# PointCloudLibrary/pcl

Hardware: AMD Instinct MI355X
Metric: ICP correspondences/sec (higher is better)
Workload: dtype f32 search / f64 accumulate

## Files before the change

### __graft_entry__.py

```python
import os
import subprocess
import sys

ROOT = os.path.dirname(os.path.abspath(__file__))
if ROOT not in sys.path:
    sys.path.insert(0, ROOT)


def build():
    env = dict(os.environ)
    env.setdefault("HIPCC", "/opt/rocm/bin/hipcc")
    subprocess.check_call(["make", "-C", os.path.join(ROOT, "pcl_amd", "csrc"), "-j8"], env=env)
    if subprocess.call(["bash", os.path.join(ROOT, "scripts", "build_variant.sh"), "verify", "-DPCLHIP_VERIFY_BOUNDS"], env=env,
                       stdout=subprocess.DEVNULL) != 0:
        print("warning: the verify-bounds variant did not build (tests/test_gpu_verify_bounds.py will skip)", file=sys.stderr)
    subprocess.check_call(["make", "-C", os.path.join(ROOT, "oracle")])
    if os.path.exists("/opt/rocm/lib/llvm/bin/clang++"):
        subprocess.check_call(["make", "-C", os.path.join(ROOT, "tests", "wavesim"), "-j8"], stdout=subprocess.DEVNULL)
    import pcl_amd
    from pcl_amd import _lib
    _lib.load()


def smoke():
    import numpy as np

    import pcl_amd
    from oracle import pcl_oracle as orc

    n = 20000
    tgt, src, T_gt = pcl_amd.synth.icp_pair(n)
    ctx = pcl_amd.Context(0)
    tree = pcl_amd.KdTree(ctx)
    tree.setInputCloud(tgt)
    gi, gd = tree.nearestKSearch(src[:4096], 8)
    otree = orc.KdTree(tgt)
    oi, od = otree.knn(src[:4096], 8)
    assert np.array_equal(gi, oi) and np.array_equal(gd, od), "k-NN mismatch vs oracle"
    ne = pcl_amd.NormalEstimation(ctx)
    ne.setInputCloud(tgt)
    ne.setSearchMethod(tree)
    ne.setKSearch(8)
    ne.setViewPoint(0, 0, 10)
    nrm = ne.compute()
    onrm, _ = otree.normals(tgt, 8, viewpoint=(0, 0, 10))
    assert np.abs(np.sum(nrm[:, :3] * onrm[:, :3], axis=1)).min() > 1 - 1e-4, "normals mismatch"
    icp = pcl_amd.IterativeClosestPointWithNormals(ctx)
    icp.setSearchMethodTarget(tree)
# ... 20 lines not shown
```

### pcl_amd/csrc/search.hip

```cpp
#include <hip/hip_runtime.h>

#include <type_traits>

#include <cfloat>
#include <cmath>
#include <cstdlib>
#include <cstring>

#include "traverse.hpp"
#include "standoff.hpp"
#include "normals_math.hpp"
#include "device_scan.hpp"
#include "icp_xform.hpp"
#include <mutex>
#include <unordered_map>
#include <vector>

namespace pclhip {

constexpr int BLOCK = 256;
constexpr int WAVES_PER_BLOCK = BLOCK / WAVE;
constexpr uint32_t COLD_RUN = 4;

#define KNN_MINW(K) ((K) <= 8 ? 4 : 1)
template <int K>
using KnnWaveLds = WaveLdsBoxT<(K == 1 ? 3072 : LEAF_BATCH * LEAF_FLOATS * 4)>;
template <int K>
__global__ __launch_bounds__(BLOCK, KNN_MINW(K)) void knn_reg_kernel(IndexView ix, const float4* __restrict__ q,
                                                        uint32_t nq, int k, int32_t* __restrict__ out_idx,
                                                        float* __restrict__ out_d2, unsigned long long* gstats) {
  __shared__ KnnWaveLds<K> wl_s[WAVES_PER_BLOCK];
  __shared__ Box topbox_s[TOPCACHE_BOXES];
  load_top_cache(ix, topbox_s);
  const int lane = threadIdx.x & (WAVE - 1);
  const uint32_t ngroups = (nq + WAVE - 1) / WAVE;
  const GroupSchedule sched(ngroups);
  TraverseStats ts;
  GroupFeed feed(sched, ix.sched_ctr);
  for (uint32_t gl = feed.first(sched); gl != GroupFeed::END; gl = feed.advance()) {
    const uint32_t g = sched.global(gl);
    if (g >= ngroups) break;
    feed.ahead(gl);
    const uint32_t i = g * WAVE + lane;
    float4 p = make_float4(0, 0, 0, 0);
    bool valid = i < nq;
    if (valid) p = q[i];
    const uint32_t oq = __float_as_uint(p.w);
    const bool real = valid;
    valid = valid && isfinite(p.x) && isfinite(p.y) && isfinite(p.z);
    const float qx[1] = {p.x}, qy[1] = {p.y}, qz[1] = {p.z};
    const bool vv[1] = {valid};
    if constexpr (K == 1) {
      NN1Min fast;
      fast.init(__builtin_inff());
      traverse<NN1Min, true>(ix, qx, qy, qz, vv, fast, wl_s[threadIdx.x / WAVE], topbox_s, ts);
// ... 716 lines not shown
__device__ __forceinline__ void icp_search_body(const IndexView& ix, float4* __restrict__ cur,
                                                const float4* __restrict__ src0, uint32_t ns, Mat34 T,
                                                const IcpControl* __restrict__ ctl, const RegionBox& region, int order,
                                                float bound, int flags, uint32_t* __restrict__ match_pos,
                                                uint32_t* __restrict__ match, float* __restrict__ match_d2,
                                                unsigned long long* gstats, IcpWaveLds* wl_s, Box* topbox_s,
                                                const OG& og = OG()) {
  static_assert(!OWNED || Q == 1, "served-group lists are per 64-point group");
  bool restart = false;
  if (ctl != nullptr) {
    if (ctl->stop != 0) return;
    restart = ctl->restart != 0;
    if ((flags & 4) != 0 && !restart) return;
#pragma unroll
    for (int i = 0; i < 12; ++i) T.m[i] = ctl->T_apply[i];
  }
  const float4* in = restart ? src0 : cur;
  const int use_max = flags & 1;
  load_top_cache(ix, topbox_s);
  const int lane = threadIdx.x & (WAVE - 1);
  const int wave = threadIdx.x / WAVE;
  const uint32_t GROUP = (Q == 1 && !OWNED) ? search_fill_of(flags) : uint32_t(WAVE * Q);
  const bool lane_in_group = (Q != 1 || OWNED) ? true : uint32_t(threadIdx.x & (WAVE - 1)) < GROUP;
  uint32_t ngroups = (ns + GROUP - 1) / GROUP;
  uint32_t epoch = 0;
  if constexpr (OWNED) {
    ngroups = og.count[0];
    epoch = og.state->epoch;
  }
  const auto gid = [&](uint32_t slot) -> uint32_t {
    if constexpr (OWNED) return slot < ngroups ? og.list[slot] : 0u;
    else return slot;
  };
  const GroupSchedule sched(ngroups);
  TraverseStats ts;
  uint32_t gl = sched.first();
  uint32_t g = (gl < sched.end()) ? sched.global(gl) : ngroups;
  GroupFeed feed(sched, ix.sched_ctr);
  const auto next_now = [&](uint32_t from) -> uint32_t {
    uint32_t out = GroupFeed::END;
    if (from == GroupFeed::END) return out;
    if (!feed.static_next(from, out)) {
      feed.request();
      out = feed.resolve();
    }
    return out;
  };
  constexpr bool deep = DEEP;
  uint32_t gl_next = (gl < sched.end()) ? next_now(gl) : GroupFeed::END;
  uint32_t gl_nn = deep ? next_now(gl_next) : GroupFeed::END;
  float4 p_n[Q], t_n[Q];
  uint32_t sp_n[Q], sp_nn[Q];
  uint32_t gid_n = gid(g), st_n = 0;
  if constexpr (OWNED) st_n = (g < ngroups && !restart) ? (og.stamp[gid_n] & 0x7FFFFFFFu) : 0u;
  {
    const uint32_t g1 = (gl_next != GroupFeed::END) ? sched.global(gl_next) : ngroups;
    const uint32_t gid1 = gid(g1);
#pragma unroll
    for (int q = 0; q < Q; ++q) {
      p_n[q] = make_float4(0, 0, 0, 0);
      t_n[q] = make_float4(0, 0, 0, 0);
      sp_n[q] = NO_INDEX;
      sp_nn[q] = NO_INDEX;
      const uint32_t i = gid_n * GROUP + q * WAVE + lane;
      if (g < ngroups && i < ns && lane_in_group) {
        p_n[q] = (OWNED && st_n == 0u) ? src0[i] : in[i];
        sp_n[q] = restart ? NO_INDEX : match_pos[i];
      }
      const uint32_t i1 = gid1 * GROUP + q * WAVE + lane;
      if (g1 < ngroups && i1 < ns && lane_in_group) sp_nn[q] = restart ? NO_INDEX : match_pos[i1];
      if (sp_n[q] != NO_INDEX) t_n[q] = ix.pts[sp_n[q]];
    }
  }
#ifdef PCLHIP_ICP_PROFILE
  uint64_t icp_t = clock64();
#define ICP_LAP(i)                              \
  do {                                          \
    const uint64_t icp_now = clock64();         \
    ts.c[i] += uint32_t(icp_now - icp_t);       \
    icp_t = icp_now;                            \
  } while (0)
#else
#define ICP_LAP(i) (void)0
#endif
  while (g < ngroups) {
    float4 p[Q], t0[Q];
    uint32_t seed_pos[Q];
    bool in_range[Q], valid[Q];
    float qx[Q], qy[Q], qz[Q];
    const uint32_t gcur = gid_n, st_cur = st_n;
#pragma unroll
    for (int q = 0; q < Q; ++q) {
      p[q] = p_n[q];
      t0[q] = t_n[q];
      seed_pos[q] = sp_n[q];
      in_range[q] = lane_in_group && (gcur * GROUP + q * WAVE + lane) < ns;
    }
    const uint32_t g2 = (gl_next != GroupFeed::END) ? sched.global(gl_next) : ngroups;
    const uint32_t g3 = (gl_nn != GroupFeed::END) ? sched.global(gl_nn) : ngroups;
    gid_n = gid(g2);
    const uint32_t gid_nn = gid(g3);
    if constexpr (OWNED) st_n = (g2 < ngroups && !restart) ? (og.stamp[gid_n] & 0x7FFFFFFFu) : 0u;
    uint32_t gl_after = GroupFeed::END;
    bool asked = false;
    const uint32_t gl_last = deep ? gl_nn : gl_next;
    if (gl_last != GroupFeed::END && !feed.static_next(gl_last, gl_after)) {
      feed.request();
      asked = true;
    }
    bool next_ok[Q];
#pragma unroll
    for (int q = 0; q < Q; ++q) {
      const uint32_t i2 = gid_n * GROUP + q * WAVE + lane;
      next_ok[q] = g2 < ngroups && i2 < ns && lane_in_group;
      p_n[q] = make_float4(0, 0, 0, 0);
      t_n[q] = make_float4(0, 0, 0, 0);
      if (deep) {
        sp_n[q] = sp_nn[q];
        if (next_ok[q]) {
          p_n[q] = (OWNED && st_n == 0u) ? src0[i2] : in[i2];
          if (sp_n[q] != NO_INDEX) t_n[q] = ix.pts[sp_n[q]];
        }
        const uint32_t i3 = gid_nn * GROUP + q * WAVE + lane;
        sp_nn[q] = NO_INDEX;
        if (g3 < ngroups && i3 < ns && lane_in_group) sp_nn[q] = restart ? NO_INDEX : match_pos[i3];
      } else {
        sp_n[q] = NO_INDEX;
        if (next_ok[q]) {
          p_n[q] = (OWNED && st_n == 0u) ? src0[i2] : in[i2];
          sp_n[q] = restart ? NO_INDEX : match_pos[i2];
        }
      }
    }
    NN1MinT<Q> fast;
    fast.init(bound);
#pragma unroll
    for (int q = 0; q < Q; ++q) {
      valid[q] = in_range[q] && isfinite(p[q].x) && isfinite(p[q].y) && isfinite(p[q].z);
      if (valid[q]) {
        if constexpr (OWNED) own_replay(og.state, st_cur, restart ? 0u : epoch, order, p[q]);
// ... 49 lines not shown
    }
#pragma unroll
    for (int q = 0; q < Q; ++q) {
      NN1 pol;
      pol.soa = ix.soa;
      pol.key = KEY_NONE;
      pol.pos = fast.bestpos[q];
      if (fast.bestpos[q] != NO_INDEX) {
        const float w = (fast.bestpos[q] == seed_pos[q]) ? t0[q].w : ix.pts[fast.bestpos[q]].w;
        pol.key = make_key(fast.best[q], __float_as_uint(w));
      }
      const bool redo[1] = {valid[q] && (fast.tie[q] || (fast.bestpos[q] == NO_INDEX && !use_max))};
      if (__builtin_amdgcn_ballot_w64(redo[0]) != 0) {
        NN1 ex = pol;
        const float ex_x[1] = {qx[q]}, ex_y[1] = {qy[q]}, ex_z[1] = {qz[q]};
        traverse<NN1, SPARSE>(ix, ex_x, ex_y, ex_z, redo, ex, wl_s[wave], topbox_s, ts);
        if (redo[0]) pol = ex;
      }
      const uint32_t mid = key_index(pol.key);
      const bool found = valid[q] && mid != NO_INDEX;
      if (in_range[q]) {
        const uint32_t i = gcur * GROUP + q * WAVE + lane;
        match[i] = found ? mid : NO_INDEX;
        match_pos[i] = found ? pol.pos : NO_INDEX;
        match_d2[i] = found ? key_dist(pol.key) : __builtin_inff();
      }
    }
    if constexpr (OWNED) {
      if (lane == 0) og.stamp[gcur] = epoch + 1u;
    }
    g = g2;
    if (deep) {
      gl_next = gl_nn;
      gl_nn = asked ? feed.resolve() : gl_after;
    } else {
      gl_next = asked ? feed.resolve() : gl_after;
    }
    ICP_LAP(7);
  }
#undef ICP_LAP
  flush_stats(ts, gstats);
}

template <bool OWNED = false, class OG = NoOwnedGroups>
__device__ __forceinline__ void icp_cold_search_body(const IndexView& ix, float4* __restrict__ cur,
                                                     const float4* __restrict__ src0, uint32_t ns, Mat34 T,
                                                     const IcpControl* __restrict__ ctl, const RegionBox& region, int order,
                                                     float bound, int flags, float so_from,
                                                     uint32_t* __restrict__ match_pos, uint32_t* __restrict__ match,
                                                     float* __restrict__ match_d2, unsigned long long* gstats,
                                                     IcpWaveLds* wl_s, Box* topbox_s, const OG& og = OG()) {
  bool restart = false;
  if (ctl != nullptr) {
    if (ctl->stop != 0) return;
    restart = true;
#pragma unroll
    for (int i = 0; i < 12; ++i) T.m[i] = ctl->T_apply[i];
  }
  const float4* in = restart ? src0 : cur;
  const int use_max = flags & 1;
  load_top_cache(ix, topbox_s);
  const int lane = threadIdx.x & (WAVE - 1);
  const int wave = threadIdx.x / WAVE;
  const uint32_t GF = OWNED ? uint32_t(WAVE) : search_fill_of(flags);
  const bool lane_in_group = uint32_t(lane) < GF;
  uint32_t ngroups = (ns + GF - 1) / GF;
  if constexpr (OWNED) ngroups = og.count[0];
  const auto gid = [&](uint32_t slot) -> uint32_t {
    if constexpr (OWNED) return slot < ngroups ? og.list[slot] : 0u;
    else return slot;
  };
  TraverseStats ts;
  PrevGroup prev;
  prev.init();
  const GroupSchedule sched(ngroups);
  constexpr uint32_t RUN = COLD_RUN;
  const uint32_t nruns = (sched.groups_per_xcd + RUN - 1u) / RUN;
  uint32_t* const run_ctr = ix.sched_ctr + (blockIdx.x % (gridDim.x < 8u ? gridDim.x : 8u)) * uint32_t(SCHED_CTR_STRIDE);
  for (uint32_t run = sched.slot_wave; run < nruns;) {
  uint32_t ticket = 0;
  if (lane == 0) ticket = atomicAdd(run_ctr, 1u);
  prev.forget();
  uint32_t gl = run * RUN;
  const uint32_t run_end = (gl + RUN) < sched.groups_per_xcd ? (gl + RUN) : sched.groups_per_xcd;
  float4 p_n = make_float4(0, 0, 0, 0);
  {
    const uint32_t g0 = (gl < run_end) ? sched.global(gl) : ngroups;
    if (g0 < ngroups && lane_in_group && gid(g0) * GF + lane < ns) p_n = in[gid(g0) * GF + lane];
  }
  for (; gl < run_end; ++gl) {
    const uint32_t g = sched.global(gl);
    if (g >= ngroups) break;
    float4 p = p_n;
    const uint32_t i = gid(g) * GF + lane;
    const bool in_range = lane_in_group && i < ns;
    {
      const uint32_t g2 = (gl + 1u < run_end) ? sched.global(gl + 1u) : ngroups;
      p_n = make_float4(0, 0, 0, 0);
      if (g2 < ngroups && lane_in_group && gid(g2) * GF + lane < ns) p_n = in[gid(g2) * GF + lane];
    }
    if constexpr (OWNED) {
      if (lane == 0) og.stamp[gid(g)] = 1u;
    }
    NN1Min fast;
    fast.init(bound);
    bool valid = in_range && isfinite(p.x) && isfinite(p.y) && isfinite(p.z);
    if (valid) {
      const float x = xform_row(T.m[0], T.m[1], T.m[2], T.m[3], p.x, p.y, p.z, order);
      const float y = xform_row(T.m[4], T.m[5], T.m[6], T.m[7], p.x, p.y, p.z, order);
      const float z = xform_row(T.m[8], T.m[9], T.m[10], T.m[11], p.x, p.y, p.z, order);
      p.x = x; p.y = y; p.z = z;
      cur[i] = p;
      if (region.on) valid = in_region(region, x, y, z);
    } else if (in_range && restart) {
      cur[i] = p;
    }
    const float qx[1] = {p.x}, qy[1] = {p.y}, qz[1] = {p.z};
    const bool vv[1] = {valid};
    uint32_t hint = NO_INDEX;
    const bool done =
        standoff_search(ix, p.x, p.y, p.z, valid, fast, wl_s[wave], topbox_s, ts, prev, (flags & 2) != 0, so_from, hint);
    prev.outcome(done);
#if defined(PCLHIP_SO_PROFILE) || defined(PCLHIP_SO_REASONS)
    const uint64_t so_t0 = clock64();
    TraverseStats ts_fb;
#else
    TraverseStats& ts_fb = ts;
#endif
    if (!done) traverse<NN1Min, true>(ix, qx, qy, qz, vv, fast, wl_s[wave], topbox_s, ts_fb, (flags & 2) ? hint : NO_INDEX, true);
    fast.resolve(ix, qx, qy, qz);
    NN1 pol;
    pol.soa = ix.soa;
    pol.key = KEY_NONE;
    pol.pos = fast.bestpos[0];
    if (fast.bestpos[0] != NO_INDEX) pol.key = make_key(fast.best[0], __float_as_uint(ix.pts[fast.bestpos[0]].w));
    {
      const bool redo[1] = {valid && (fast.tie[0] || (fast.bestpos[0] == NO_INDEX && !use_max))};
      if (__builtin_amdgcn_ballot_w64(redo[0]) != 0) {
        NN1 ex = pol;
        traverse<NN1, true>(ix, qx, qy, qz, redo, ex, wl_s[wave], topbox_s, ts_fb);
        if (redo[0]) pol = ex;
      }
    }
    const uint32_t mid = key_index(pol.key);
    const bool found = valid && mid != NO_INDEX;
    if (in_range) {
      match[i] = found ? mid : NO_INDEX;
      match_pos[i] = found ? pol.pos : NO_INDEX;
      match_d2[i] = found ? key_dist(pol.key) : __builtin_inff();
    }
    prev.record(p.x, p.y, p.z, found ? pol.pos : NO_INDEX);
#if defined(PCLHIP_SO_PROFILE)
    ts.c[7] += uint32_t(clock64() - so_t0);
    if (!done) ++ts.c[4];
#elif defined(PCLHIP_SO_REASONS)
    (void)so_t0;
    if (!done) ++ts.c[4];
#endif
  }
  run = sched.waves_per_xcd + uniform_u32(ticket);
  }
  flush_stats(ts, gstats);
}

template <int MINW, int Q, bool SPARSE, bool DEEP = false>
__global__ __launch_bounds__(BLOCK, MINW) void icp_search_kernel(IndexView ix, float4* __restrict__ cur,
                                                                 const float4* __restrict__ src0, uint32_t ns,
                                                                 Mat34 T, const IcpControl* __restrict__ ctl,
                                                                 RegionBox region, int order, float bound, int flags,
                                                                 uint32_t* __restrict__ match_pos,
                                                                 uint32_t* __restrict__ match,
                                                                 float* __restrict__ match_d2,
                                                                 unsigned long long* gstats
                                                                 ) {
  __shared__ IcpWaveLds wl_s[WAVES_PER_BLOCK];
  __shared__ Box topbox_s[TOPCACHE_BOXES];
  icp_search_body<Q, SPARSE, false, NoOwnedGroups, DEEP>(ix, cur, src0, ns, T, ctl, region, order, bound, flags, match_pos, match,
                                                         match_d2, gstats, wl_s, topbox_s);
}

#ifndef PCLHIP_COLD_MINW
#define PCLHIP_COLD_MINW 4
#endif
__global__ __launch_bounds__(BLOCK, PCLHIP_COLD_MINW) void icp_cold_search_kernel(
    IndexView ix, float4* __restrict__ cur, const float4* __restrict__ src0, uint32_t ns, Mat34 T,
    const IcpControl* __restrict__ ctl, RegionBox region, int order, float bound, int flags, float so_from,
    uint32_t* __restrict__ match_pos, uint32_t* __restrict__ match, float* __restrict__ match_d2, unsigned long long* gstats) {
  __shared__ IcpWaveLds wl_s[WAVES_PER_BLOCK];
  __shared__ Box topbox_s[TOPCACHE_BOXES];
  icp_cold_search_body(ix, cur, src0, ns, T, ctl, region, order, bound, flags, so_from, match_pos, match, match_d2, gstats,
                       wl_s, topbox_s);
}

template <bool DEEP>
// ... 758 lines not shown
    }
    (void)hipEventRecord(device_loop ? ev[0] : icp->ev0, s);
    if (lane_now && !device_loop) {
    } else if (owned) {
      hipLaunchKernelGGL(icp_own_flag_kernel, dim3((ngroups + BLOCK - 1) / BLOCK), dim3(BLOCK), 0, s, ctl, icp->own_state,
                         icp->own_gbox, icp->region, ngroups, icp->n, icp->own_stamp, icp->own_flags, icp->own_prefix, icp->match,
                         icp->match_pos, icp->match_d2);
      hipLaunchKernelGGL(icp_own_list_kernel, dim3((ngroups + OWN_CHUNK - 1) / OWN_CHUNK), dim3(BLOCK), 0, s, ctl, icp->own_state,
                         icp->own_flags, icp->own_prefix, ngroups, icp->own_list, icp->own_tot);
      const int go = resident_blocks(ctx, icp_search_owned_kernel, ngroups);
      PCLHIP_LAUNCH_FED(ctx, icp_search_owned_kernel, dim3(go), dim3(BLOCK), 0, s, v, icp->src_cur, icp->src_sorted0, icp->n, M,
                         ctl, icp->region, order, bound, kflags, so_from, standoff ? 1 : 0, icp->match_pos, icp->match,
                         icp->match_d2, ctx->stats, og);
    } else if (standoff && device_loop) {
      const int gd = resident_blocks(ctx, icp_search_dual_kernel<false>, ngroups);
      if (deep_for(gd, ngroups)) {
        PCLHIP_LAUNCH_FED(ctx, icp_search_dual_kernel<true>, dim3(gd), dim3(BLOCK), 0, s, v, icp->src_cur, icp->src_sorted0, icp->n, M,
                           ctl, icp->region, order, bound, kflags, so_from, icp->match_pos, icp->match, icp->match_d2, ctx->stats);
      } else {
        PCLHIP_LAUNCH_FED(ctx, icp_search_dual_kernel<false>, dim3(gd), dim3(BLOCK), 0, s, v, icp->src_cur, icp->src_sorted0, icp->n, M,
                           ctl, icp->region, order, bound, kflags, so_from, icp->match_pos, icp->match, icp->match_d2, ctx->stats);
      }
    } else if (cold) {
      const int gc = resident_blocks(ctx, icp_cold_search_kernel, ngroups);
      PCLHIP_LAUNCH_FED(ctx, icp_cold_search_kernel, dim3(gc), dim3(BLOCK), 0, s, v, icp->src_cur, icp->src_sorted0, icp->n, M,
                         ctl, icp->region, order, bound, kflags, so_from, icp->match_pos, icp->match, icp->match_d2,
                         ctx->stats);
    } else {
      const int gk = resident_blocks(ctx, ks, ngroups);
      if (deep_for(gk, ngroups)) ks = icp_search_kernel<4, 1, true, true>;
      PCLHIP_LAUNCH_FED(ctx, ks, dim3(gk), dim3(BLOCK), 0, s, v, icp->src_cur, icp->src_sorted0,
                         icp->n, M, ctl, icp->region, order, bound, kflags, icp->match_pos, icp->match, icp->match_d2, ctx->stats);
    }
    if (lane_now) {
      const pclhip_status lst = launch_lane_search(icp, M.m, ctl, order, bound, use_max);
      if (lst != PCLHIP_OK) return lst;
    }
    (void)hipEventRecord(device_loop ? ev[1] : icp->ev_mid, s);
    icp->mid_recorded = true;
    if (icp->search_only && !device_loop) {
      (void)hipEventRecord(icp->ev1, s);
      PCLHIP_CHECK_HIP(ctx, hipGetLastError());
      return PCLHIP_OK;
    }
    const uint8_t* keep = nullptr;
    if (filters) {
      pclhip_status st = apply_correspondence_filters(icp, max_d2, use_max);
      if (st != PCLHIP_OK) return st;
      keep = icp->keep;
    }
    constexpr int acc_per_cu = 4;
    int ga = ctx->num_cus * acc_per_cu;
    if (ga > icp->grid_blocks) ga = icp->grid_blocks;
    {
      const int need = int((uint64_t(icp->n) + 1023u) / 1024u);
      if (ga > need) ga = need < 64 ? 64 : need;
    }
    if (owned && mode == PCLHIP_ICP_POINT_TO_PLANE)
      hipLaunchKernelGGL(icp_accumulate_owned_kernel<PCLHIP_ICP_POINT_TO_PLANE>, dim3(ga), dim3(BLOCK), 0, s, v, icp->src_cur,
                         icp->n, icp->match_pos, icp->match_d2, keep, ctl, icp->enforce_same_direction_normals ? 1 : 0,
                         icp->partials, og);
    else if (owned)
      hipLaunchKernelGGL(icp_accumulate_owned_kernel<PCLHIP_ICP_POINT_TO_POINT>, dim3(ga), dim3(BLOCK), 0, s, v, icp->src_cur,
                         icp->n, icp->match_pos, icp->match_d2, keep, ctl, icp->enforce_same_direction_normals ? 1 : 0,
                         icp->partials, og);
    else if (mode == PCLHIP_ICP_POINT_TO_PLANE)
      launch_accumulate<PCLHIP_ICP_POINT_TO_PLANE>(icp, v, ga, keep, M, ctl, s);
    else if (mode == PCLHIP_ICP_SYMMETRIC)
      launch_accumulate<PCLHIP_ICP_SYMMETRIC>(icp, v, ga, keep, M, ctl, s);
    else
      launch_accumulate<PCLHIP_ICP_POINT_TO_POINT>(icp, v, ga, keep, M, ctl, s);
    (void)hipEventRecord(device_loop ? ev[2] : icp->ev1, s);
    solved = device_loop && !icp_is_sharded(icp);
    hipLaunchKernelGGL(icp_finalize_kernel, dim3(1), dim3(FINALIZE_THREADS), 0, s, icp->partials, ga, icp->sums_dev, ctl,
                       solved ? icp->ctl : static_cast<IcpControl*>(nullptr), icp->steps);
  } else {
    if (device_loop) {
      (void)hipEventRecord(ev[0], s);
      (void)hipEventRecord(ev[1], s);
    }
    if (filters) {
      const pclhip_status es = apply_empty_shard_collectives(icp);
      if (es != PCLHIP_OK) return es;
    }
    PCLHIP_CHECK_HIP(ctx, hipMemsetAsync(icp->sums_dev, 0, NS * sizeof(double), s));
    if (device_loop) (void)hipEventRecord(ev[2], s);
  }
  PCLHIP_CHECK_HIP(ctx, hipGetLastError());
  pclhip_status st = allreduce_record(icp);
// ... 119 lines not shown
  PCLHIP_CHECK_HIP(ctx, e);
  return PCLHIP_OK;
}

int icp_grid_blocks(pclhip_ctx* ctx, uint32_t ns) {
  const uint32_t ngroups = (ns + WAVE - 1) / WAVE;
  int g = resident_blocks(ctx, icp_search_kernel<4, 1, true>, ngroups);
  if (ctx->num_cus * 8 > g) g = ctx->num_cus * 8;
  return g;
}


bool search_built_with_verify_bounds() {
#ifdef PCLHIP_VERIFY_BOUNDS
  return true;
#else
  return false;
#endif
}

void preload_search_kernels(pclhip_ctx* ctx) {
  (void)resident_blocks(ctx, icp_search_kernel<4, 1, true>, 1);
  (void)resident_blocks(ctx, icp_cold_search_kernel, 1);
  (void)resident_blocks(ctx, icp_search_dual_kernel<false>, 1);
  (void)resident_blocks(ctx, icp_search_dual_kernel<true>, 1);
  (void)resident_blocks(ctx, icp_search_kernel<4, 1, true, true>, 1);
  (void)resident_blocks(ctx, normals_kernel<8>, 1);
  (void)resident_blocks(ctx, knn_reg_kernel<1>, 1);
}

}

#include "gicp.hpp"
```

### pcl_amd/csrc/traverse.hpp

```cpp
#pragma once

#include "pclhip_internal.hpp"

namespace pclhip {

constexpr int STACK_ENTRIES = 208;
constexpr int LEAF_BATCH = 16;
#ifndef PCLHIP_PAIR_MODE
#define PCLHIP_PAIR_MODE 1
#endif
constexpr bool pair_mode = PCLHIP_PAIR_MODE != 0;
constexpr int LEAF_FLOATS = 4 * LEAF;

template <int BUF_BYTES>
struct __attribute__((aligned(16))) WaveLdsT {
  static constexpr int BUF_FLOATS = BUF_BYTES / 4;
  static constexpr int LIST_STRIDE = 3;
  uint2 stack[STACK_ENTRIES];
  float4 list[3 * FANOUT];
  float rad[FANOUT];
  float buf[BUF_FLOATS];
  __device__ __forceinline__ float* radii() { return rad; }
};
template <int BUF_BYTES>
// ... 1109 lines not shown
      } else if (alive && lane != jn) {
        const int at = sp + __builtin_popcountll(others & ((1ull << lane) - 1ull));
        stack[at] = make_uint2((cl << 28) | (first + uint32_t(lane)), __float_as_uint(lbG));
      }
      sp += __builtin_popcountll(others);
#ifndef PCLHIP_STATS_LANES
      ts.c[3] += uint32_t(__builtin_popcountll(others));
#endif
      __builtin_amdgcn_wave_barrier();
      level = cl;
      node = first + uint32_t(jn);
      have = true;
    }
  }
}

__device__ __forceinline__ void flush_stats(const TraverseStats& ts_in, unsigned long long* g) {
#ifdef PCLHIP_VERIFY_BOUNDS
  TraverseStats ts = ts_in;
#pragma unroll
  for (int o = 32; o > 0; o >>= 1) {
    ts.c[6] += __shfl_xor(ts.c[6], o);
    ts.c[7] += __shfl_xor(ts.c[7], o);
  }
#else
  const TraverseStats& ts = ts_in;
#endif
  if (g != nullptr && (threadIdx.x & (WAVE - 1)) == 0) {
#pragma unroll
    for (int i = 0; i < 8; ++i) atomicAdd(g + i, (unsigned long long)ts.c[i]);
  }
}

struct GroupSchedule {
  uint32_t groups_per_xcd, xcd_first, slot_wave, waves_per_xcd;
  __device__ __forceinline__ GroupSchedule(uint32_t ngroups) {
    const uint32_t nxcd = gridDim.x < 8u ? gridDim.x : 8u;
    const uint32_t xcd = blockIdx.x % nxcd, slot = blockIdx.x / nxcd;
    const uint32_t slots = (gridDim.x + nxcd - 1 - xcd) / nxcd;
    const uint32_t waves_per_block = blockDim.x / WAVE;
    groups_per_xcd = (ngroups + nxcd - 1) / nxcd;
    xcd_first = xcd * groups_per_xcd;
    slot_wave = slot * waves_per_block + threadIdx.x / WAVE;
    waves_per_xcd = slots * waves_per_block;
  }
  __device__ __forceinline__ uint32_t first() const { return slot_wave; }
  __device__ __forceinline__ uint32_t step() const { return waves_per_xcd; }
  __device__ __forceinline__ uint32_t end() const { return groups_per_xcd; }
  __device__ __forceinline__ uint32_t global(uint32_t g) const { return xcd_first + g; }
};

struct GroupFeed {
  static constexpr uint32_t END = 0xFFFFFFFFu;
  uint32_t step_, static_end_, end_;
  uint32_t* ctr_;
  uint32_t ticket_, next_;
  bool asked_;
  __device__ __forceinline__ GroupFeed(const GroupSchedule& s, uint32_t* counters) {
    step_ = s.step();
    end_ = s.end();
#ifndef PCLHIP_DYN_STATIC_8THS
#define PCLHIP_DYN_STATIC_8THS 4
#endif
    const uint32_t all = end_ / step_;
    uint32_t rounds = all * uint32_t(PCLHIP_DYN_STATIC_8THS) / 8u;
    if (rounds < 1u) rounds = 1u;
    static_end_ = (counters != nullptr && all >= 2u) ? rounds * step_ : end_;
    const uint32_t nxcd = gridDim.x < 8u ? gridDim.x : 8u;
    ctr_ = counters + (blockIdx.x % nxcd) * uint32_t(SCHED_CTR_STRIDE);
    ticket_ = 0;
    next_ = END;
    asked_ = false;
  }
  __device__ __forceinline__ uint32_t first(const GroupSchedule& s) const { return s.first() < end_ ? s.first() : END; }
  __device__ __forceinline__ uint32_t strides() const { return end_ / step_; }
  __device__ __forceinline__ bool static_next(uint32_t gl, uint32_t& out) const {
    if (static_end_ == end_) {
      out = (gl + step_ < end_) ? gl + step_ : END;
      return true;
    }
    if (gl < static_end_ && gl + step_ < static_end_) {
      out = gl + step_;
      return true;
    }
    return false;
  }
  __device__ __forceinline__ void request() {
    if ((threadIdx.x & (WAVE - 1)) == 0) ticket_ = atomicAdd(ctr_, 1u);
  }
  __device__ __forceinline__ uint32_t resolve() const {
    const uint32_t g = static_end_ + uniform_u32(ticket_);
    return g < end_ ? g : END;
  }
  __device__ __forceinline__ void ahead(uint32_t gl) {
    asked_ = !static_next(gl, next_);
    if (asked_) request();
  }
  __device__ __forceinline__ uint32_t advance() const { return asked_ ? resolve() : next_; }
};

}
```

Measured before the change: 10.71 billion.

## Add interleaved XCD chunk windows and cross-XCD work stealing to ICP search

```diff
diff --git a/__graft_entry__.py b/__graft_entry__.py
--- a/__graft_entry__.py
+++ b/__graft_entry__.py
@@ -14,6 +14,10 @@
     if subprocess.call(["bash", os.path.join(ROOT, "scripts", "build_variant.sh"), "verify", "-DPCLHIP_VERIFY_BOUNDS"], env=env,
                        stdout=subprocess.DEVNULL) != 0:
         print("warning: the verify-bounds variant did not build (tests/test_gpu_verify_bounds.py will skip)", file=sys.stderr)
+    if subprocess.call(["bash", os.path.join(ROOT, "scripts", "build_variant.sh"), "audit",
+                        "-DPCLHIP_SCHED_AUDIT -DPCLHIP_ICP_SEEDED_BALANCE=1"], env=env,
+                       stdout=subprocess.DEVNULL) != 0:
+        print("warning: the schedule-audit variant did not build (tests/test_gpu_icp_schedule.py will fail)", file=sys.stderr)
     subprocess.check_call(["make", "-C", os.path.join(ROOT, "oracle")])
     if os.path.exists("/opt/rocm/lib/llvm/bin/clang++"):
         subprocess.check_call(["make", "-C", os.path.join(ROOT, "tests", "wavesim"), "-j8"], stdout=subprocess.DEVNULL)
diff --git a/pcl_amd/csrc/search.hip b/pcl_amd/csrc/search.hip
--- a/pcl_amd/csrc/search.hip
+++ b/pcl_amd/csrc/search.hip
@@ -21,6 +21,76 @@
 constexpr int BLOCK = 256;
 constexpr int WAVES_PER_BLOCK = BLOCK / WAVE;
 constexpr uint32_t COLD_RUN = 4;
+#ifndef PCLHIP_ICP_CHUNK_ROUNDS
+#define PCLHIP_ICP_CHUNK_ROUNDS 1
+#endif
+#ifndef PCLHIP_ICP_STEAL
+#define PCLHIP_ICP_STEAL 1
+#endif
+#ifndef PCLHIP_ICP_SEEDED_BALANCE
+#define PCLHIP_ICP_SEEDED_BALANCE 0
+#endif
+constexpr uint32_t ICP_CHUNK_ROUNDS = PCLHIP_ICP_CHUNK_ROUNDS;
+constexpr bool ICP_STEAL = PCLHIP_ICP_STEAL != 0;
+constexpr bool ICP_SEEDED_BALANCE = PCLHIP_ICP_SEEDED_BALANCE != 0 && (ICP_CHUNK_ROUNDS != 0u || ICP_STEAL);
+
+#ifdef PCLHIP_XCD_PROFILE
+constexpr uint32_t XCD_PROF_LAUNCHES = 16, XCD_PROF_WAVES = 8192;
+struct XcdProfRec {
+  unsigned long long t_first, t_exit;
+  uint32_t xcc, label, groups, stolen;
+};
+__device__ XcdProfRec g_xcd_prof[XCD_PROF_LAUNCHES][XCD_PROF_WAVES];
+__device__ uint32_t g_xcd_prof_launch;
+__global__ void xcd_prof_next_kernel() { g_xcd_prof_launch = g_xcd_prof_launch + 1u; }
+struct SchedProbe {
+  unsigned long long t_first = 0;
+  uint32_t groups = 0, stolen = 0;
+  __device__ __forceinline__ void group(uint32_t, bool, bool was_stolen) {
+    if (groups == 0u) t_first = wall_clock64();
+    ++groups;
+    if (was_stolen) ++stolen;
+  }
+  __device__ __forceinline__ void exit() {
+    const unsigned long long now = wall_clock64();
+    const uint32_t w = blockIdx.x * (blockDim.x / WAVE) + threadIdx.x / WAVE;
+    if ((threadIdx.x & (WAVE - 1)) == 0 && w < XCD_PROF_WAVES) {
+      XcdProfRec r;
+      r.t_first = groups != 0u ? t_first : now;
+      r.t_exit = now;
+      r.xcc = uint32_t(__builtin_amdgcn_s_getreg(20 | (3 << 11))) & 15u;
+      r.label = blockIdx.x % (gridDim.x < 8u ? gridDim.x : 8u);
+      r.groups = groups;
+      r.stolen = stolen;
+      g_xcd_prof[g_xcd_prof_launch % XCD_PROF_LAUNCHES][w] = r;
+    }
+  }
+};
+#elif defined(PCLHIP_SCHED_AUDIT)
+constexpr uint32_t SCHED_AUDIT_GROUPS = 1u << 18;
+__device__ uint32_t g_sched_audit[SCHED_AUDIT_GROUPS + 4];
+struct SchedProbe {
+  __device__ __forceinline__ void group(uint32_t g, bool cold, bool was_stolen) {
+    if ((threadIdx.x & (WAVE - 1)) == 0) {
+      if (g < SCHED_AUDIT_GROUPS) atomicAdd(&g_sched_audit[g], 1u);
+      atomicAdd(&g_sched_audit[SCHED_AUDIT_GROUPS + (cold ? 1u : 0u)], 1u);
+      if (was_stolen) atomicAdd(&g_sched_audit[SCHED_AUDIT_GROUPS + (cold ? 3u : 2u)], 1u);
+    }
+  }
+  __device__ __forceinline__ void exit() {}
+};
+__global__ void sched_audit_fetch_kernel(uint32_t* out) {
+  for (uint32_t i = blockIdx.x * blockDim.x + threadIdx.x; i < SCHED_AUDIT_GROUPS + 4u; i += gridDim.x * blockDim.x) {
+    out[i] = g_sched_audit[i];
+    g_sched_audit[i] = 0u;
+  }
+}
+#else
+struct SchedProbe {
+  __device__ __forceinline__ void group(uint32_t, bool, bool) {}
+  __device__ __forceinline__ void exit() {}
+};
+#endif
 
 #define KNN_MINW(K) ((K) <= 8 ? 4 : 1)
 template <int K>
@@ -803,17 +873,18 @@
     if constexpr (OWNED) return slot < ngroups ? og.list[slot] : 0u;
     else return slot;
   };
-  const GroupSchedule sched(ngroups);
+  const GroupSchedule sched = !ICP_SEEDED_BALANCE ? GroupSchedule(ngroups) : GroupSchedule(ngroups, ICP_CHUNK_ROUNDS, COLD_RUN);
   TraverseStats ts;
+  SchedProbe prof;
   uint32_t gl = sched.first();
   uint32_t g = (gl < sched.end()) ? sched.global(gl) : ngroups;
-  GroupFeed feed(sched, ix.sched_ctr);
+  std::conditional_t<ICP_SEEDED_BALANCE, StealFeed<ICP_STEAL>, OwnFeed> feed(sched, ix.sched_ctr);
   const auto next_now = [&](uint32_t from) -> uint32_t {
     uint32_t out = GroupFeed::END;
     if (from == GroupFeed::END) return out;
     if (!feed.static_next(from, out)) {
-      feed.request();
-      out = feed.resolve();
+      feed.request(sched);
+      out = feed.resolve(sched);
     }
     return out;
   };
@@ -825,7 +896,7 @@
   uint32_t gid_n = gid(g), st_n = 0;
   if constexpr (OWNED) st_n = (g < ngroups && !restart) ? (og.stamp[gid_n] & 0x7FFFFFFFu) : 0u;
   {
-    const uint32_t g1 = (gl_next != GroupFeed::END) ? sched.global(gl_next) : ngroups;
+    const uint32_t g1 = (gl_next != GroupFeed::END) ? feed.global_of(sched, gl_next) : ngroups;
     const uint32_t gid1 = gid(g1);
 #pragma unroll
     for (int q = 0; q < Q; ++q) {
@@ -860,6 +931,7 @@
     bool in_range[Q], valid[Q];
     float qx[Q], qy[Q], qz[Q];
     const uint32_t gcur = gid_n, st_cur = st_n;
+    prof.group(g, false, sched.win.owner(g) != sched.xcd);
 #pragma unroll
     for (int q = 0; q < Q; ++q) {
       p[q] = p_n[q];
@@ -867,8 +939,8 @@
       seed_pos[q] = sp_n[q];
       in_range[q] = lane_in_group && (gcur * GROUP + q * WAVE + lane) < ns;
     }
-    const uint32_t g2 = (gl_next != GroupFeed::END) ? sched.global(gl_next) : ngroups;
-    const uint32_t g3 = (gl_nn != GroupFeed::END) ? sched.global(gl_nn) : ngroups;
+    const uint32_t g2 = (gl_next != GroupFeed::END) ? feed.global_of(sched, gl_next) : ngroups;
+    const uint32_t g3 = (gl_nn != GroupFeed::END) ? feed.global_of(sched, gl_nn) : ngroups;
     gid_n = gid(g2);
     const uint32_t gid_nn = gid(g3);
     if constexpr (OWNED) st_n = (g2 < ngroups && !restart) ? (og.stamp[gid_n] & 0x7FFFFFFFu) : 0u;
@@ -876,7 +948,7 @@
     bool asked = false;
     const uint32_t gl_last = deep ? gl_nn : gl_next;
     if (gl_last != GroupFeed::END && !feed.static_next(gl_last, gl_after)) {
-      feed.request();
+      feed.request(sched);
       asked = true;
     }
     bool next_ok[Q];
@@ -992,13 +1064,14 @@
     g = g2;
     if (deep) {
       gl_next = gl_nn;
-      gl_nn = asked ? feed.resolve() : gl_after;
+      gl_nn = asked ? feed.resolve(sched) : gl_after;
     } else {
-      gl_next = asked ? feed.resolve() : gl_after;
+      gl_next = asked ? feed.resolve(sched) : gl_after;
     }
     ICP_LAP(7);
   }
 #undef ICP_LAP
+  prof.exit();
   flush_stats(ts, gstats);
 }
 
@@ -1033,29 +1106,21 @@
   TraverseStats ts;
   PrevGroup prev;
   prev.init();
-  const GroupSchedule sched(ngroups);
   constexpr uint32_t RUN = COLD_RUN;
-  const uint32_t nruns = (sched.groups_per_xcd + RUN - 1u) / RUN;
-  uint32_t* const run_ctr = ix.sched_ctr + (blockIdx.x % (gridDim.x < 8u ? gridDim.x : 8u)) * uint32_t(SCHED_CTR_STRIDE);
-  for (uint32_t run = sched.slot_wave; run < nruns;) {
-  uint32_t ticket = 0;
-  if (lane == 0) ticket = atomicAdd(run_ctr, 1u);
+  SchedProbe prof;
+  const auto search_run = [&](uint32_t run_first, uint32_t run_len, bool run_taken) {
   prev.forget();
-  uint32_t gl = run * RUN;
-  const uint32_t run_end = (gl + RUN) < sched.groups_per_xcd ? (gl + RUN) : sched.groups_per_xcd;
+  const uint32_t run_end = run_first + run_len;
   float4 p_n = make_float4(0, 0, 0, 0);
-  {
-    const uint32_t g0 = (gl < run_end) ? sched.global(gl) : ngroups;
-    if (g0 < ngroups && lane_in_group && gid(g0) * GF + lane < ns) p_n = in[gid(g0) * GF + lane];
-  }
-  for (; gl < run_end; ++gl) {
-    const uint32_t g = sched.global(gl);
+  if (run_first < ngroups && lane_in_group && gid(run_first) * GF + lane < ns) p_n = in[gid(run_first) * GF + lane];
+  for (uint32_t g = run_first; g < run_end; ++g) {
     if (g >= ngroups) break;
+    prof.group(g, true, run_taken);
     float4 p = p_n;
     const uint32_t i = gid(g) * GF + lane;
     const bool in_range = lane_in_group && i < ns;
     {
-      const uint32_t g2 = (gl + 1u < run_end) ? sched.global(gl + 1u) : ngroups;
+      const uint32_t g2 = (g + 1u < run_end) ? g + 1u : ngroups;
       p_n = make_float4(0, 0, 0, 0);
       if (g2 < ngroups && lane_in_group && gid(g2) * GF + lane < ns) p_n = in[gid(g2) * GF + lane];
     }
@@ -1118,8 +1183,43 @@
     if (!done) ++ts.c[4];
 #endif
   }
-  run = sched.waves_per_xcd + uniform_u32(ticket);
-  }
+  };
+  if constexpr (ICP_CHUNK_ROUNDS == 0u && !ICP_STEAL) {
+    const GroupSchedule sched(ngroups);
+    const uint32_t nruns = (sched.groups_per_xcd + RUN - 1u) / RUN;
+    uint32_t* const run_ctr = ix.sched_ctr + sched.xcd * uint32_t(SCHED_CTR_STRIDE);
+    for (uint32_t run = sched.slot_wave; run < nruns;) {
+      uint32_t ticket = 0;
+      if (lane == 0) ticket = atomicAdd(run_ctr, 1u);
+      const uint32_t gl = run * RUN;
+      search_run(sched.global(gl), (gl + RUN) < sched.groups_per_xcd ? RUN : sched.groups_per_xcd - gl, false);
+      run = sched.waves_per_xcd + uniform_u32(ticket);
+    }
+  } else {
+    const GroupSchedule sched(ngroups, ICP_CHUNK_ROUNDS, RUN);
+    const auto own_run = [&](uint32_t run, uint32_t& len) -> uint32_t {
+      const uint32_t e = sched.groups_per_xcd, gl = run * RUN;
+      len = gl >= e ? 0u : (gl + RUN < e ? RUN : e - gl);
+      return len != 0u ? sched.global(gl) : 0u;
+    };
+    uint32_t state = sched.xcd;
+    uint32_t run_len = 0;
+    uint32_t run_first = own_run(sched.slot_wave, run_len);
+    while (run_len != 0u) {
+      uint32_t ticket = 0;
+      if (lane == 0) ticket = atomicAdd(ix.sched_ctr + (state & 15u) * uint32_t(SCHED_CTR_STRIDE), 1u);
+      search_run(run_first, run_len, sched.win.owner(run_first) != sched.xcd);
+      run_len = 0u;
+      if ((state & 15u) == sched.xcd) run_first = own_run(sched.waves_per_xcd + uniform_u32(ticket), run_len);
+      if (run_len == 0u && (ICP_STEAL || (state & 15u) != sched.xcd) && (state & 15u) < sched.win.nxcd) {
+        const StolenWork w = steal_resolve<ICP_STEAL>(ix.sched_ctr, sched.win, sched.xcd, RUN, state, uniform_u32(ticket));
+        state = w.state;
+        run_first = w.first;
+        run_len = w.count;
+      }
+    }
+  }
+  prof.exit();
   flush_stats(ts, gstats);
 }
 
@@ -1944,6 +2044,9 @@
       PCLHIP_LAUNCH_FED(ctx, ks, dim3(gk), dim3(BLOCK), 0, s, v, icp->src_cur, icp->src_sorted0,
                          icp->n, M, ctl, icp->region, order, bound, kflags, icp->match_pos, icp->match, icp->match_d2, ctx->stats);
     }
+#ifdef PCLHIP_XCD_PROFILE
+    hipLaunchKernelGGL(xcd_prof_next_kernel, dim3(1), dim3(1), 0, s);
+#endif
     if (lane_now) {
       const pclhip_status lst = launch_lane_search(icp, M.m, ctl, order, bound, use_max);
       if (lst != PCLHIP_OK) return lst;
@@ -1967,6 +2070,7 @@
     {
       const int need = int((uint64_t(icp->n) + 1023u) / 1024u);
       if (ga > need) ga = need < 64 ? 64 : need;
+      if (ga > icp->grid_blocks) ga = icp->grid_blocks;
     }
     if (owned && mode == PCLHIP_ICP_POINT_TO_PLANE)
       hipLaunchKernelGGL(icp_accumulate_owned_kernel<PCLHIP_ICP_POINT_TO_PLANE>, dim3(ga), dim3(BLOCK), 0, s, v, icp->src_cur,
@@ -2152,3 +2256,44 @@
 }
 
 #include "gicp.hpp"
+
+#ifdef PCLHIP_XCD_PROFILE
+extern "C" PCLHIP_API int pclhip_xcd_profile_read(void* out, int launches_cap, int waves, int reset) {
+  if (hipDeviceSynchronize() != hipSuccess) return -1;
+  uint32_t n = 0;
+  if (hipMemcpyFromSymbol(&n, HIP_SYMBOL(pclhip::g_xcd_prof_launch), sizeof(n)) != hipSuccess) return -1;
+  int got = int(n < pclhip::XCD_PROF_LAUNCHES ? n : pclhip::XCD_PROF_LAUNCHES);
+  if (got > launches_cap) got = launches_cap;
+  if (waves > int(pclhip::XCD_PROF_WAVES)) waves = int(pclhip::XCD_PROF_WAVES);
+  for (int l = 0; out != nullptr && l < got; ++l)
+    if (hipMemcpyFromSymbol(static_cast<char*>(out) + size_t(l) * size_t(waves) * sizeof(pclhip::XcdProfRec),
+                            HIP_SYMBOL(pclhip::g_xcd_prof), size_t(waves) * sizeof(pclhip::XcdProfRec),
+                            size_t(l) * sizeof(pclhip::XcdProfRec) * pclhip::XCD_PROF_WAVES) != hipSuccess)
+      return -1;
+  if (reset != 0) {
+    void* p = nullptr;
+    n = 0;
+    if (hipMemcpyToSymbol(HIP_SYMBOL(pclhip::g_xcd_prof_launch), &n, sizeof(n)) != hipSuccess) return -1;
+    if (hipGetSymbolAddress(&p, HIP_SYMBOL(pclhip::g_xcd_prof)) != hipSuccess) return -1;
+    if (hipMemset(p, 0, sizeof(pclhip::XcdProfRec) * pclhip::XCD_PROF_LAUNCHES * pclhip::XCD_PROF_WAVES) != hipSuccess) return -1;
+  }
+  return got;
+}
+#endif
+
+#ifdef PCLHIP_SCHED_AUDIT
+extern "C" PCLHIP_API int pclhip_sched_audit_fetch(uint32_t* visits, uint32_t groups, uint32_t* totals) {
+  constexpr uint32_t N = pclhip::SCHED_AUDIT_GROUPS + 4u;
+  if (groups > pclhip::SCHED_AUDIT_GROUPS) return -1;
+  uint32_t* dev = nullptr;
+  if (hipDeviceSynchronize() != hipSuccess || hipMalloc(reinterpret_cast<void**>(&dev), N * sizeof(uint32_t)) != hipSuccess) return -1;
+  hipLaunchKernelGGL(pclhip::sched_audit_fetch_kernel, dim3(64), dim3(256), 0, nullptr, dev);
+  std::vector<uint32_t> host(N);
+  const bool ok = hipMemcpy(host.data(), dev, N * sizeof(uint32_t), hipMemcpyDeviceToHost) == hipSuccess;
+  (void)hipFree(dev);
+  if (!ok) return -1;
+  if (visits != nullptr) std::memcpy(visits, host.data(), size_t(groups) * sizeof(uint32_t));
+  if (totals != nullptr) std::memcpy(totals, host.data() + pclhip::SCHED_AUDIT_GROUPS, 4 * sizeof(uint32_t));
+  return 0;
+}
+#endif
diff --git a/pcl_amd/csrc/traverse.hpp b/pcl_amd/csrc/traverse.hpp
--- a/pcl_amd/csrc/traverse.hpp
+++ b/pcl_amd/csrc/traverse.hpp
@@ -1165,22 +1165,65 @@
   }
 }
 
+struct XcdWindows {
+  uint32_t ngroups, nxcd;
+  uint32_t window;
+  uint32_t shift;
+  __device__ __forceinline__ uint32_t groups_of(uint32_t x) const {
+    if (window != 0u) {
+      const uint32_t first = x * window;
+      return first >= ngroups ? 0u : (ngroups - first < window ? ngroups - first : window);
+    }
+    const uint32_t nchunks = (ngroups + (1u << shift) - 1u) >> shift;
+    if (x >= nchunks) return 0u;
+    const uint32_t mine = (nchunks - x + nxcd - 1u) / nxcd;
+    const uint32_t ragged = ((nchunks - 1u) % nxcd == x) ? (nchunks << shift) - ngroups : 0u;
+    return (mine << shift) - ragged;
+  }
+  __device__ __forceinline__ uint32_t global(uint32_t x, uint32_t gl) const {
+    return window != 0u ? x * window + gl : ((((gl >> shift) * nxcd + x) << shift) | (gl & ((1u << shift) - 1u)));
+  }
+  __device__ __forceinline__ uint32_t owner(uint32_t g) const { return window != 0u ? g / window : (g >> shift) % nxcd; }
+  __device__ __forceinline__ uint32_t waves_of(uint32_t x) const {
+    return ((gridDim.x + nxcd - 1u - x) / nxcd) * (blockDim.x / WAVE);
+  }
+};
+
 struct GroupSchedule {
   uint32_t groups_per_xcd, xcd_first, slot_wave, waves_per_xcd;
+  XcdWindows win;
+  uint32_t xcd;
   __device__ __forceinline__ GroupSchedule(uint32_t ngroups) {
     const uint32_t nxcd = gridDim.x < 8u ? gridDim.x : 8u;
-    const uint32_t xcd = blockIdx.x % nxcd, slot = blockIdx.x / nxcd;
+    xcd = blockIdx.x % nxcd;
+    const uint32_t slot = blockIdx.x / nxcd;
     const uint32_t slots = (gridDim.x + nxcd - 1 - xcd) / nxcd;
     const uint32_t waves_per_block = blockDim.x / WAVE;
     groups_per_xcd = (ngroups + nxcd - 1) / nxcd;
     xcd_first = xcd * groups_per_xcd;
     slot_wave = slot * waves_per_block + threadIdx.x / WAVE;
     waves_per_xcd = slots * waves_per_block;
+    win.ngroups = ngroups;
+    win.nxcd = nxcd;
+    win.window = groups_per_xcd != 0u ? groups_per_xcd : 1u;
+    win.shift = 0u;
+  }
+  __device__ __forceinline__ GroupSchedule(uint32_t ngroups, uint32_t chunk_rounds, uint32_t run) : GroupSchedule(ngroups) {
+    const uint32_t nxcd = win.nxcd;
+    const uint32_t want = chunk_rounds * run * ((gridDim.x + nxcd - 1u) / nxcd) * (blockDim.x / WAVE);
+    if (want != 0u) {
+      const uint32_t shift = 32u - uint32_t(__builtin_clz(want - 1u | 1u));
+      if (((ngroups + (1u << shift) - 1u) >> shift) >= 2u * nxcd) {
+        win.window = 0u;
+        win.shift = shift;
+      }
+    }
+    groups_per_xcd = win.groups_of(xcd);
   }
   __device__ __forceinline__ uint32_t first() const { return slot_wave; }
   __device__ __forceinline__ uint32_t step() const { return waves_per_xcd; }
   __device__ __forceinline__ uint32_t end() const { return groups_per_xcd; }
-  __device__ __forceinline__ uint32_t global(uint32_t g) const { return xcd_first + g; }
+  __device__ __forceinline__ uint32_t global(uint32_t g) const { return win.window != 0u ? xcd_first + g : win.global(xcd, g); }
 };
 
 struct GroupFeed {
@@ -1195,15 +1238,18 @@
 #ifndef PCLHIP_DYN_STATIC_8THS
 #define PCLHIP_DYN_STATIC_8THS 4
 #endif
-    const uint32_t all = end_ / step_;
-    uint32_t rounds = all * uint32_t(PCLHIP_DYN_STATIC_8THS) / 8u;
-    if (rounds < 1u) rounds = 1u;
-    static_end_ = (counters != nullptr && all >= 2u) ? rounds * step_ : end_;
+    static_end_ = static_end_of(end_, step_, counters != nullptr);
     const uint32_t nxcd = gridDim.x < 8u ? gridDim.x : 8u;
     ctr_ = counters + (blockIdx.x % nxcd) * uint32_t(SCHED_CTR_STRIDE);
     ticket_ = 0;
     next_ = END;
     asked_ = false;
+  }
+  static __device__ __forceinline__ uint32_t static_end_of(uint32_t end, uint32_t step, bool fed) {
+    const uint32_t all = end / step;
+    uint32_t rounds = all * uint32_t(PCLHIP_DYN_STATIC_8THS) / 8u;
+    if (rounds < 1u) rounds = 1u;
+    return (fed && all >= 2u) ? rounds * step : end;
   }
   __device__ __forceinline__ uint32_t first(const GroupSchedule& s) const { return s.first() < end_ ? s.first() : END; }
   __device__ __forceinline__ uint32_t strides() const { return end_ / step_; }
@@ -1232,4 +1278,94 @@
   __device__ __forceinline__ uint32_t advance() const { return asked_ ? resolve() : next_; }
 };
 
-}
+template <class Supply>
+__device__ __forceinline__ uint32_t next_victim(uint32_t* counters, uint32_t nxcd, uint32_t own, uint32_t& dead,
+                                                const Supply& supply_of) {
+  const uint32_t lane = threadIdx.x & (WAVE - 1);
+  bool has = false;
+  if (lane < nxcd && ((dead >> lane) & 1u) == 0u) has = atomicAdd(counters + lane * uint32_t(SCHED_CTR_STRIDE), 0u) < supply_of(lane);
+  const uint32_t live = uint32_t(__builtin_amdgcn_ballot_w64(has));
+  dead |= ~live;
+  for (uint32_t k = 1; k < nxcd; ++k) {
+    const uint32_t v = (own + k) % nxcd;
+    if ((live >> v) & 1u) return v;
+  }
+  return nxcd;
+}
+
+struct StolenWork {
+  uint32_t first, count, state;
+};
+template <bool STEAL>
+__device__ __attribute__((noinline)) StolenWork steal_resolve(uint32_t* counters, XcdWindows win, uint32_t own, uint32_t run,
+                                                              uint32_t state, uint32_t ticket) {
+  const auto take = [&](uint32_t v, uint32_t t, StolenWork& w) -> bool {
+    const uint32_t e = win.groups_of(v);
+    const uint32_t gl = run == 0u ? GroupFeed::static_end_of(e, win.waves_of(v), true) + t : (win.waves_of(v) + t) * run;
+    if (gl >= e) return false;
+    w.first = win.global(v, gl);
+    w.count = run == 0u ? 1u : (e - gl < run ? e - gl : run);
+    return true;
+  };
+  StolenWork w;
+  uint32_t v = state & 15u, dead = state >> 8;
+  w.state = state;
+  if (take(v, ticket, w)) return w;
+  if (STEAL) {
+    for (;;) {
+      dead |= 1u << v;
+      v = next_victim(counters, win.nxcd, own, dead, [&](uint32_t x) -> uint32_t {
+        const uint32_t e = win.groups_of(x);
+        if (run == 0u) return e - GroupFeed::static_end_of(e, win.waves_of(x), true);
+        const uint32_t r = (e + run - 1u) / run, wv = win.waves_of(x);
+        return r > wv ? r - wv : 0u;
+      });
+      if (v >= win.nxcd) break;
+      uint32_t t = 0;
+      if ((threadIdx.x & (WAVE - 1)) == 0) t = atomicAdd(counters + v * uint32_t(SCHED_CTR_STRIDE), 1u);
+      w.state = v | ((dead & 0xFFu) << 8);
+      if (take(v, uniform_u32(t), w)) return w;
+    }
+  }
+  w.first = GroupFeed::END;
+  w.count = 0u;
+  w.state = win.nxcd;
+  return w;
+}
+
+struct OwnFeed : GroupFeed {
+  __device__ __forceinline__ OwnFeed(const GroupSchedule& s, uint32_t* counters) : GroupFeed(s, counters) {}
+  __device__ __forceinline__ uint32_t global_of(const GroupSchedule& s, uint32_t gl) const { return s.global(gl); }
+  __device__ __forceinline__ void request(const GroupSchedule&) { GroupFeed::request(); }
+  __device__ __forceinline__ uint32_t resolve(const GroupSchedule&) const { return GroupFeed::resolve(); }
+};
+
+template <bool STEAL>
+struct StealFeed : GroupFeed {
+  static constexpr uint32_t STOLEN = 0x80000000u;
+  uint32_t state_;
+  __device__ __forceinline__ StealFeed(const GroupSchedule& s, uint32_t* counters) : GroupFeed(s, counters) { state_ = s.xcd; }
+  __device__ __forceinline__ uint32_t global_of(const GroupSchedule& s, uint32_t gl) const {
+    return (gl & STOLEN) != 0u ? (gl & ~STOLEN) : s.global(gl);
+  }
+  __device__ __forceinline__ void request(const GroupSchedule& s) {
+    const uint32_t v = state_ & 15u;
+    if (v < s.win.nxcd && (threadIdx.x & (WAVE - 1)) == 0)
+      ticket_ = atomicAdd(ctr_ + (int(v) - int(s.xcd)) * SCHED_CTR_STRIDE, 1u);
+  }
+  __device__ __forceinline__ uint32_t resolve(const GroupSchedule& s) {
+    const uint32_t v = state_ & 15u;
+    if (v >= s.win.nxcd) return END;
+    const uint32_t t = uniform_u32(ticket_);
+    if (v == s.xcd && static_end_ + t < end_) return static_end_ + t;
+    if (v == s.xcd && !STEAL) {
+      state_ = s.win.nxcd;
+      return END;
+    }
+    const StolenWork w = steal_resolve<STEAL>(ctr_ - int(s.xcd) * SCHED_CTR_STRIDE, s.win, s.xcd, 0u, state_, t);
+    state_ = w.state;
+    return w.first == END ? END : (STOLEN | w.first);
+  }
+};
+
+}
```

New measurement: 10.57 billion. -1.3%, worse.
